# fizzy74/passport-zk-circuits

Hardware: AMD Instinct MI355X
Metric: registerIdentityBuilder witnesses/sec, batch=4096, 1 & 8 MI355X; % HBM roofline (higher is better)
Workload: dtype bn254_fr (u32 limbs)

## Files before the change

passport-zk-circuits_amd/csrc/builder_ecdsa.cpp:

```cpp
#include "builder_impl.hpp"
#include "ec_walk.hpp"

namespace pzk {

namespace {

struct EcSym { int idx = -1; };

struct EcProgCtx {
  using V = EcSym;
  uint32_t* d;
  uint32_t size;
  uint32_t n = 0;
  bool bad = false;
  uint32_t& at(uint32_t off) {
    static uint32_t sink;
    if (off >= size) { bad = true; return sink; }
    return d[off];
  }
  V put(uint32_t off, const V&) { at(off) = ecd(ECD_COPY, n); return V{(int)n++}; }
  V put_hidden(const V&) { return V{(int)n++}; }
  void cp(uint32_t off, const V& v) {
    if (v.idx < 0) bad = true;
    else at(off) = ecd(ECD_COPY, (uint32_t)v.idx);
// ... 22 lines not shown
  void check_one(const V&) const {}
  int nl = 4;
  void div_signed(const V*, int, int MCN, V& sign, V* k) const {
    sign = {};
    for (int i = 0; i < MCN - nl + 1; i++) k[i] = {};
  }
  void divmod_n(const V*, V* q, V* r) const {
    for (int i = 0; i < nl + 1; i++) q[i] = {};
    for (int i = 0; i < nl; i++) r[i] = {};
  }
};

template <int CV>
bool ec_program(int t, std::vector<uint32_t>& P, uint32_t& n) {
  const uint32_t size = ec_type_size(EC_GEO[CV], t);
  P.assign(size, ecd(ECD_ZERO, 0));
  EcProgCtx c{P.data(), size};
  c.nl = EC_GEO[CV].nl;
  EcWalk<EcProgCtx, CV> walk(c);
  walk.run(t);
  n = c.n;
  return !c.bad;
}

uint32_t sz_n2b(int L) { return 2 * L + 1; }

}

bool ec_programs(Layout& L, std::string& why) {
  const int cv = L.reg.ec_curve;
  const EcGeo& G = EC_GEO[cv];
  L.ec_prog.clear();
  for (int t = 0; t < ECT_N; t++) {
    std::vector<uint32_t> P;
    uint32_t n = 0;
    const bool ok = cv == 0 ? ec_program<0>(t, P, n) : cv == 1 ? ec_program<1>(t, P, n) : cv == 2 ? ec_program<2>(t, P, n)
                                                                                         : ec_program<3>(t, P, n);
    if (!ok || n > EC_TABLE_MAX[cv]) {
      why = "internal: ECDSA table program " + std::to_string(t) +
            (!ok ? " addresses a signal outside its block" : " too large (" + std::to_string(n) + " entries)");
      return false;
    }
    L.ec_prog_off[t] = (uint32_t)L.ec_prog.size();
    L.ec_tab_n[t] = n;
    L.ec_prog.insert(L.ec_prog.end(), P.begin(), P.end());
  }
  L.ec_tab_off.clear();
  for (int i = 0; i < ECT_N; i++) L.ec_ops[i].clear();
  uint32_t off = 0;
  for (int t = 0; t < G.n_ops + EC_N_MM; t++) {
    const int type = t >= G.n_ops ? ECT_MM : ec_op_is_dbl(G, t) ? ECT_DBL : ECT_ADD;
    L.ec_tab_off.push_back(off);
    L.ec_ops[type].push_back(t);
    off += L.ec_tab_n[type];
  }
  L.ec_tab_entries = off;
  return true;
}

void ec_verify_regions(Builder& b, int cv, int IN_PK, int IN_SIG, int J_SA) {
  const EcGeo& G = EC_GEO[cv];
  const int N = G.nl, CS = G.cs, F = G.fb, P2 = 2 * N;
  auto ect = [&](int t, int type) { b.region(RK_ECT, ec_type_size(G, type), {t, type}); };
  auto ecop = [&](int op) { ect(op, ec_op_is_dbl(G, op) ? ECT_DBL : ECT_ADD); };
  b.region(RK_INCOPY, P2, {IN_PK});
  b.region(RK_INCOPY, P2, {IN_SIG});
  b.region(RK_DIGEST, F, {J_SA});
  b.region(RK_INCOPY, P2, {IN_PK});
  b.region(RK_INCOPY, P2, {IN_SIG});
  b.region(RK_DIGEST, F, {J_SA});
  b.region(RK_HCHUNK, N, {J_SA, N, CS});
  b.region(RK_EC_CONST, N, {EC_K_ONE});
  b.region(RK_EC_CONST, N, {EC_K_ORDER});
  b.region(RK_EC_U64, N, {G.c_sinv});
  for (int i = 0; i < N; i++) b.region(RK_BITS2NUM, sz_n2b(CS), {CS, 1, i * CS + CS - 1, -1, J_SA});
  b.region(RK_EC_CONST, N, {EC_K_ORDER});
  b.region(RK_EC_U64, N, {G.c_sinv});
  b.region(RK_INCOPY, N, {IN_SIG + N});
  b.region(RK_EC_CONST, N, {EC_K_ORDER});
  ect(G.n_ops + EC_MM_INV, ECT_MM);
  ect(G.n_ops + EC_MM_U1, ECT_MM);
  ect(G.n_ops + EC_MM_U2, ECT_MM);
  b.region(RK_EC_U64, P2, {G.c_gm_rp + P2 * (G.parts - 2)});
  b.region(RK_EC_U64, N, {G.c_u1});
  b.region(RK_EC_GM_RCC, (uint64_t)G.parts * 256 * P2);
  b.region(RK_EC_U64, G.parts * P2, {G.c_gm_ap});
  b.region(RK_VALUE, 4 * G.parts * P2, {-2});
  b.region(RK_EC_U64, (G.parts - 1) * P2, {G.c_gm_rp});
  b.region(RK_VALUE, P2, {-2});
  for (int i = 0; i < N; i++) b.region(RK_EC_N2B, sz_n2b(CS), {0, G.c_u1 + i, CS});
  b.region(RK_EC_B2N8, G.parts * 17, {G.c_u1});
  b.region(RK_EC_CONST, P2, {EC_K_DUMMY});
  ecop(EC_OP_SD);
  b.region(RK_EC_GM_EQ, (uint64_t)G.parts * 256 * 6);
  b.region(RK_EC_GM_SUM, (uint64_t)G.parts * P2 * 512);
  for (int i = 0; i < G.parts - 1; i++) {
    ecop(ec_op_gm_add(i));
    b.region(RK_EC_GM_STEP, 4 * 6 + 2 * P2 * 6, {i});
  }
  b.region(RK_EC_U64, P2, {G.c_sm_rp + P2 * G.wins});
  b.region(RK_INCOPY, P2, {IN_PK});
  b.region(RK_EC_U64, N, {G.c_u2});
  b.region(RK_EC_SBITS, F, {G.c_u2});
  b.region(RK_EC_U64, (G.wins + 1) * P2, {G.c_sm_rp});
  b.region(RK_EC_U64, G.wins * P2, {G.c_sm_ap});
  b.region(RK_EC_U64, 16 * P2, {G.c_pre});
  b.region(RK_INCOPY, P2, {IN_PK});
// ... 23 lines not shown
```

passport-zk-circuits_amd/csrc/ec_common.hpp:

```cpp
#pragma once
#include <hip/hip_runtime.h>
#include <stdint.h>

namespace pzk {

constexpr int EC_N_CURVES = 4;
constexpr int EC_MAXN = 7;
__host__ __device__ constexpr int ec_curve_of_sig(int sig) {
  return sig == 20 ? 0 : sig == 21 ? 1 : sig == 24 ? 2 : sig == 25 ? 3 : -1;
}
constexpr int EC_NL[EC_N_CURVES] = {4, 4, 7, 6};
constexpr int EC_CS[EC_N_CURVES] = {64, 64, 32, 64};

constexpr uint64_t EC_CURVE_K[EC_N_CURVES][5][2 * EC_MAXN] = {
    {{18446744073709551612ull, 4294967295ull, 0ull, 18446744069414584321ull},
     {4309448131093880907ull, 7285987128567378166ull, 12964664127075681980ull, 6540974713487397863ull},
     {18446744073709551615ull, 4294967295ull, 0ull, 18446744069414584321ull},
     {17562291160714782033ull, 13611842547513532036ull, 18446744073709551615ull, 18446744069414584320ull},
     {4148137498610012746ull, 51237685452122967ull, 6555942389409504868ull, 799804747332166731ull,
      13395177781894339167ull, 1107697421929919296ull, 6228258783500845564ull, 11862546499924939746ull}},
    {{16810331318623712729ull, 18122579188607900780ull, 17219079075415130087ull, 9032542404991529047ull},
     {7767825457231955894ull, 10773760575486288334ull, 17523706096862592191ull, 2800214691157789508ull},
     {2311270323689771895ull, 7943213001558335528ull, 4496292894210231666ull, 12248480212390422972ull},
     {10384753744809580199ull, 10104242082523752183ull, 4496292894210231665ull, 12248480212390422972ull},
// ... 48 lines not shown
  const int P2 = 2 * N;
  g.c_sinv = 0; g.c_u1 = N; g.c_u2 = 2 * N; g.c_h = 3 * N;
  g.c_mm = 4 * N;
  g.c_gm_ap = g.c_mm + 4 * P2;
  g.c_gm_rp = g.c_gm_ap + g.parts * P2;
  g.c_pre = g.c_gm_rp + (g.parts - 1) * P2;
  g.c_sm_ap = g.c_pre + 16 * P2;
  g.c_sm_rp = g.c_sm_ap + g.wins * P2;
  g.c_rec = g.c_sm_rp + (g.wins + 1) * P2;
  g.rec_words = 3 * P2;
  g.core_words = g.c_rec + g.n_ops * g.rec_words;
  g.i_sm_zr = 4 * (g.parts - 1);
  g.i_sm_za = g.i_sm_zr + g.wins;
  g.n_inv = g.i_sm_za + g.wins - 1;
  g.n_pts = g.parts + (g.parts - 1) + 16 + g.wins + (g.wins + 1);
  g.jw = (g.fb + 63) / 64;
  g.j_op = (3 * g.jw + 2) & ~1;
  g.j_pts = g.n_ops * g.j_op;
  g.jac_words = g.j_pts + (g.n_pts + 1) / 2;
  g.sz_poncurve = P2 + 3 * ec_bmo(N, N) + ec_bmo(2 * N - 1, N) + ec_bizmp(cs, N, 3 * cs + 2 * N, 3 * N - 2, 3 * N);
  g.sz_pontangent = 4 * N + ec_bmo(N, N) + (2 * (2 * N - 1) + 1) + (2 * (2 * N - 1) + N) + 4 * N + ec_bmo(2 * N - 1, N) +
                    (2 * N + 1) + 3 * N + ec_bmo(N, N) + ec_bizmp(cs, N, 3 * cs + 2 * N, 3 * N - 2, 3 * N + 1);
  g.sz_ponline = 6 * N + 3 * N + 3 * 4 * N + 2 * ec_bmo(N, N) + ec_bizmp(cs, N, 2 * cs + 2 * N, 2 * N - 1, 2 * N + 1);
  g.sz_dbl = 4 * N + g.sz_pontangent + g.sz_poncurve;
  g.sz_add = 6 * N + g.sz_poncurve + g.sz_ponline;
  g.sz_blet = 1 + 2 * N + N + N * ((3 + ec_n2b(cs + 1)) + 6);
  g.sz_mm = (N + 1) + N + 3 * N + ec_bmo(N, N) + N * ec_n2b(cs) + (1 + 2 * N + g.sz_blet) + ec_bmneq(N + 1, N) +
            ec_bisz(cs, 2 * cs + ec_log_ceil(2 * N), 2 * N - 1);
  return g;
}
constexpr EcGeo EC_GEO[EC_N_CURVES] = {ec_geo_make(4, 64), ec_geo_make(4, 64), ec_geo_make(7, 32), ec_geo_make(6, 64)};
static_assert(EC_GEO[0].n_ops == 362 && EC_GEO[2].n_ops == 318 && EC_GEO[3].n_ops == 538, "EC op counts");

constexpr int EC_OP_SD = 0;
__host__ __device__ constexpr int ec_op_gm_add(int i) { return 1 + i; }
__host__ __device__ constexpr int ec_op_pre(const EcGeo& G, int i) { return G.parts + (i - 2); }
__host__ __device__ constexpr int ec_op_sm_dbl(const EcGeo& G, int d) { return G.op_sm0 + (d / 4) * 5 + (d % 4); }
__host__ __device__ constexpr int ec_op_sm_add(const EcGeo& G, int a) { return G.op_sm0 + a * 5 + 4; }
__host__ __device__ constexpr bool ec_op_is_dbl(const EcGeo& G, int op) {
  return op == EC_OP_SD || (op >= G.parts && op < G.op_sm0 && (op - G.parts) % 2 == 0) ||
         (op >= G.op_sm0 && op < G.op_final && (op - G.op_sm0) % 5 != 4);
}
enum { EC_MM_INV = 0, EC_MM_U1 = 1, EC_MM_U2 = 2, EC_MM_XN = 3, EC_N_MM = 4 };

enum : uint32_t { ECD_ZERO = 0, ECD_COPY = 1, ECD_BIT = 2, ECD_MASK = 3 };
__host__ __device__ constexpr uint32_t ecd(uint32_t op, uint32_t idx, uint32_t bit = 0) {
  return (op << 29) | (bit << 20) | idx;
}
enum EcType { ECT_DBL = 0, ECT_ADD = 1, ECT_MM = 2, ECT_N = 3 };
__host__ __device__ constexpr uint32_t ec_type_size(const EcGeo& G, int t) {
  return t == ECT_DBL ? G.sz_dbl : t == ECT_ADD ? G.sz_add : G.sz_mm;
}
constexpr uint32_t EC_TABLE_MAX[EC_N_CURVES] = {640, 640, 1600, 1216};

#ifndef PZK_EC_CURVE
#define PZK_EC_CURVE 0
#endif
#if PZK_EC_CURVE == 0
#define PZK_EC_NS ec_c0
#elif PZK_EC_CURVE == 1
#define PZK_EC_NS ec_c1
#elif PZK_EC_CURVE == 2
#define PZK_EC_NS ec_c2
#else
#define PZK_EC_NS ec_c3
#endif
inline namespace PZK_EC_NS {
static constexpr int EC_CV = PZK_EC_CURVE;
static constexpr EcGeo ECG = EC_GEO[EC_CV];
static constexpr const uint64_t (&EC_A)[2 * EC_MAXN] = EC_CURVE_K[EC_CV][EC_K_A];
static constexpr const uint64_t (&EC_B)[2 * EC_MAXN] = EC_CURVE_K[EC_CV][EC_K_B];
static constexpr const uint64_t (&EC_P)[2 * EC_MAXN] = EC_CURVE_K[EC_CV][EC_K_P];
static constexpr const uint64_t (&EC_N)[2 * EC_MAXN] = EC_CURVE_K[EC_CV][EC_K_ORDER];
static constexpr const uint64_t (&EC_D)[2 * EC_MAXN] = EC_CURVE_K[EC_CV][EC_K_DUMMY];
}

}
```

passport-zk-circuits_amd/csrc/ec_core.hpp:

```cpp
#pragma once
#include "ec_common.hpp"
#include "ec_walk.hpp"
#include "fr.hpp"
#include "layout.hpp"
#include "core_util.hpp"
#include "mapsink.hpp"
#include "bufs.hpp"
#include "ec_emit.hpp"

namespace pzk {
inline namespace PZK_EC_NS {

static constexpr int NL = ECG.nl, CS = ECG.cs, P2 = 2 * ECG.nl;
static constexpr int NW = (ECG.fb + 31) / 32, JW = ECG.jw;
static constexpr uint64_t CS_MASK = CS == 64 ? ~0ull : (1ull << CS) - 1;

struct I256 { uint32_t w[8]; };
__device__ __forceinline__ I256 i_u64(uint64_t x) {
  I256 r; r.w[0] = (uint32_t)x; r.w[1] = (uint32_t)(x >> 32);
#pragma unroll
  for (int i = 2; i < 8; i++) r.w[i] = 0;
  return r;
}
__device__ __forceinline__ I256 i_pow2(int k) {
// ... 92 lines not shown
      } else break;
    }
    uint64_t carry = 0, borrow = 0;
#pragma unroll
    for (int i = 0; i < NB; i++) {
      uint64_t pl = qhat * v[i], ph = __umul64hi(qhat, v[i]);
      pl += carry; ph += pl < carry;
      uint64_t t = u[i + j] - pl;
      uint64_t b1 = u[i + j] < pl;
      uint64_t t2 = t - borrow;
      b1 += t < borrow;
      u[i + j] = t2; borrow = b1; carry = ph;
    }
    uint64_t t = u[j + NB] - carry, b1 = u[j + NB] < carry;
    uint64_t t2 = t - borrow; b1 += t < borrow;
    u[j + NB] = t2;
    if (b1) {
      qhat--;
      uint64_t c = 0;
#pragma unroll
      for (int i = 0; i < NB; i++) {
        uint64_t s1 = u[i + j] + v[i], c1 = s1 < v[i];
        uint64_t s2 = s1 + c; c1 += s2 < c;
        u[i + j] = s2; c = c1;
      }
      u[j + NB] += c;
    }
    q[j] = qhat;
  }
#pragma unroll
  for (int i = 0; i < NB; i++) r[i] = (u[i] >> s) | (s ? u[i + 1] << (64 - s) : 0);
}
__device__ __forceinline__ void chunks_to_words(const uint64_t* ch, int n, uint64_t* w, int nw) {
  for (int i = 0; i < nw; i++) w[i] = 0;
  for (int i = 0; i < n; i++) w[(CS * i) >> 6] |= ch[i] << ((CS * i) & 63);
}
__device__ __forceinline__ uint64_t word_chunk(const uint64_t* w, int i) {
  return (w[(CS * i) >> 6] >> ((CS * i) & 63)) & CS_MASK;
}
static constexpr int PWORDS = (ECG.fb + 63) / 64;
__device__ __forceinline__ void const_words(const uint64_t* ch, uint64_t* w) { chunks_to_words(ch, NL, w, PWORDS); }

template <int AW32>
__device__ __forceinline__ void acc_signed(uint32_t* acc, const I256& v, int i) {
  const int off = (CS / 32) * i;
  const uint32_t ext = i_is_neg(v) ? ~0u : 0u;
  uint64_t c = 0;
  for (int j = 0; off + j < AW32; j++) {
    const uint64_t s = (uint64_t)acc[off + j] + (j < 8 ? v.w[j] : ext) + c;
    acc[off + j] = (uint32_t)s; c = s >> 32;
  }
}

struct EcTabCtx {
  using V = I256;
  uint4* tab;
  uint32_t n;
  const uint64_t* rp;
  int32_t err;
  __device__ void fail(int32_t code) { if (!err || code < err) err = code; }
  __device__ void store(const V& v) {
    I256 f = i_to_fr(v);
    tab[2 * n] = make_uint4(f.w[0], f.w[1], f.w[2], f.w[3]);
    tab[2 * n + 1] = make_uint4(f.w[4], f.w[5], f.w[6], f.w[7]);
    n++;
  }
  __device__ V put(uint32_t, const V& v) { store(v); return v; }
  __device__ V put_hidden(const V& v) { store(v); return v; }
  __device__ void cp(uint32_t, const V&) {}
  __device__ void bits(uint32_t, const V& v, int L) { if (!i_fits(v, L)) fail(ST_NUM2BITS); }
  __device__ void masks(uint32_t, const V&, int) {}
  __device__ V u64(uint64_t x) const { return i_u64(x); }
  __device__ V pow2(int k) const { return i_pow2(k); }
  __device__ V add(const V& a, const V& b) const { return i_add(a, b); }
  __device__ V sub(const V& a, const V& b) const { return i_sub(a, b); }
  __device__ V mul(const V& a, const V& b) const { return i_mul(a, b); }
  __device__ V neg(const V& a) const { return i_neg(a); }
  __device__ V sel(const V& c, const V& a, const V& b) const { return c.w[0] ? a : b; }
  __device__ V is_zero(const V& a) const { return i_u64(i_is_zero(a) ? 1 : 0); }
  __device__ V bit(const V& a, int b) const { return i_u64(i_bit(a, b)); }
  __device__ V shr_exact(const V& t, int) {
    I256 r; const uint32_t s = i_is_neg(t) ? ~0u : 0u;
    if (CS == 64) {
      if (t.w[0] | t.w[1]) fail(ST_BIGISZERO);
      return i_shr64(t);
    }
    if (t.w[0]) fail(ST_BIGISZERO);
#pragma unroll
    for (int i = 0; i < 8; i++) r.w[i] = i + 1 < 8 ? t.w[i + 1] : s;
    return r;
  }
  __device__ V inv_fr(const V& d) const {
    fr x = fr_mul_fast(i_as_fr(i_to_fr(d)), fr_const(R2_));
    fr y = fr_from_mont_fast(fr_inv<true>(x));
    I256 r;
    for (int i = 0; i < 8; i++) r.w[i] = y.v[i];
    return r;
  }
  __device__ void check_zero(const V& v) { if (!i_is_zero(v)) fail(ST_BIGISZERO); }
  __device__ void check_one(const V& v) {
    if (!i_is_zero(i_sub(v, i_u64(1)))) fail(ST_BIGMOD_GT);
  }
  __device__ void div_signed(const V* in, int CN, int MCN, V& sign, V* k) {
    constexpr int AW = ((3 * NL + 1) * CS + 63) / 64 + 2, AW32 = 2 * AW;
    uint32_t acc[AW32];
    for (int i = 0; i < AW32; i++) acc[i] = 0;
    for (int i = 0; i < CN; i++) acc_signed<AW32>(acc, in[i], i);
    const bool pos = !(acc[AW32 - 1] >> 31);
    if (!pos) {
      uint64_t c = 1;
      for (int i = 0; i < AW32; i++) { const uint64_t x = (uint64_t)(uint32_t)~acc[i] + c; acc[i] = (uint32_t)x; c = x >> 32; }
    }
    uint64_t a[AW], pw[PWORDS], q[AW], r[PWORDS];
    for (int i = 0; i < AW; i++) { a[i] = (uint64_t)acc[2 * i + 1] << 32 | acc[2 * i]; q[i] = 0; }
    const_words(EC_P, pw);
    const int na = (MCN * CS + 63) / 64;
    mp_divmod<PWORDS>(a, na < PWORDS ? PWORDS : na, pw, q, r);
    sign = i_u64(pos ? 1 : 0);
    for (int i = 0; i < MCN - NL + 1; i++) k[i] = i_u64(word_chunk(q, i));
// ... 548 lines not shown
    if (ec_op_is_dbl(ECG, it)) { for (int i = 0; i < P2; i++) rc[P2 + i] = 0; }
    else aff((int32_t)(uint32_t)(hh >> 32), rc + P2);
  } else if (it < ECG.n_ops + ECG.n_pts) {
    const int idx = it - ECG.n_ops;
    aff(reinterpret_cast<const int32_t*>(J + ECG.j_pts)[idx], C + ec_pt_base(idx));
  } else {
    const uint64_t* x1 = C + ECG.c_rec + ECG.rec_words * ECG.op_final + 2 * P2;
    eW xm = m_reduce<ModN>(ew_from_chunks(x1).v, 0);
    uint64_t xr[NL];
    ew_to_chunks(xm, xr);
    bool ok = true;
    for (int i = 0; i < NL; i++) {
      ok &= xr[i] == *reinterpret_cast<const uint64_t*>(row + 32ull * (L.reg.in_sig + i));
      C[ECG.c_mm + P2 * EC_MM_XN + i] = x1[i];
      C[ECG.c_mm + P2 * EC_MM_XN + NL + i] = i == 0 ? 1 : 0;
    }
    if (!ok && status) lane_status(status + w, ST_ECDSA_R);
  }
}

__device__ __forceinline__ fr ec_inv_diff(const uint64_t* ec_core, uint32_t w, int j) {
  const uint64_t* C = ec_core + (size_t)w * ECG.core_words;
  const uint64_t dx = EC_D[0];
  fr d;
  if (j < ECG.i_sm_zr) {
    const int i = j >> 2, k = j & 3;
    const uint64_t lx = i == 0 ? C[ECG.c_gm_ap] : C[ECG.c_gm_rp + P2 * (i - 1)], rx = C[ECG.c_gm_ap + P2 * (i + 1)];
    const uint64_t sdx = C[ECG.c_rec + ECG.rec_words * EC_OP_SD + 2 * P2];
    d = fr_diff_u64(k < 2 ? lx : rx, (k & 1) ? sdx : dx);
  } else if (j < ECG.i_sm_za) {
    d = fr_diff_u64(dx, C[ECG.c_sm_rp + P2 * (j - ECG.i_sm_zr)]);
  } else {
    d = fr_diff_u64(dx, C[ECG.c_sm_ap + P2 * (j - ECG.i_sm_za + 1)]);
  }
  return d;
}

__global__ void __launch_bounds__(64) k_ec_inv(const uint64_t* ec_core, fr* ec_inv, uint32_t batch) {
  const uint32_t gid = blockIdx.x * blockDim.x + threadIdx.x;
  const uint32_t w = gid / ECG.n_inv;
  const int j = (int)(gid % ECG.n_inv);
  const bool live = w < batch;
  fr d = fr_zero();
  if (live) d = ec_inv_diff(ec_core, w, j);
  const fr a = fr_is_zero(d) ? fr_mont_one() : fr_mul_fast(d, fr_const(R2_));
  fr others, total;
  fr_group_others<64>(a, others, total);
  const fr r = fr_mul_fast(fr_inv<true>(total), others);
  if (live) ec_inv[(size_t)w * ECG.n_inv + j] = fr_is_zero(d) ? d : fr_from_mont_fast(r);
}


template <int TYPE>
__global__ void __launch_bounds__(64) k_ec_table(DevLayout L, const int32_t* ops, const uint64_t* ec_core, uint8_t* ec_tab,
                                                 int32_t* status, uint32_t batch) {
  const uint32_t w = blockIdx.x * blockDim.x + threadIdx.x;
  if (w >= batch) return;
  const int t = ops[blockIdx.y];
  const uint64_t* C = ec_core + (size_t)w * ECG.core_words;
  const uint64_t* rec = t < ECG.n_ops ? C + ECG.c_rec + ECG.rec_words * t : C + ECG.c_mm + P2 * (t - ECG.n_ops);
  uint4* tab = reinterpret_cast<uint4*>(ec_tab + 32ull * ((size_t)w * L.ec_tab_entries + L.ec_tab_off[t]));
  EcTabCtx c{tab, 0, rec, 0};
  EcWalk<EcTabCtx, EC_CV> walk(c);
  walk.run(TYPE);
  if (c.err && status) lane_status(status + w, c.err);
}

__device__ __forceinline__ uint4 ect_value(const uint4* tab, uint32_t d, uint32_t half) {
  const uint32_t op = d >> 29, bit = (d >> 20) & 511u, idx = d & 0xfffffu;
  if (op == ECD_ZERO) return make_uint4(0u, 0u, 0u, 0u);
  if (op == ECD_COPY) return tab[2 * idx + half];
  if (op == ECD_BIT) {
    if (half) return make_uint4(0u, 0u, 0u, 0u);
    const uint4 q = tab[2 * idx + (bit >> 7)];
    const uint32_t k = (bit >> 5) & 3u, wv = k == 0 ? q.x : k == 1 ? q.y : k == 2 ? q.z : q.w;
    return make_uint4((wv >> (bit & 31u)) & 1u, 0u, 0u, 0u);
  }
  const uint4 q = tab[2 * idx + half];
  const int nb = (int)bit + 1, lo = 128 * (int)half;
  auto mw = [&](uint32_t x, int k) -> uint32_t {
    const int b0 = lo + 32 * k;
    return nb >= b0 + 32 ? x : nb <= b0 ? 0u : (x & ((1u << (nb - b0)) - 1u));
  };
  return make_uint4(mw(q.x, 0), mw(q.y, 1), mw(q.z, 2), mw(q.w, 3));
}

constexpr int ECT_NT = EC_TABLE_MAX[EC_CV] > 1024 ? 512 : 256;
template <int MM, int ECT_U>
__global__ void __launch_bounds__(ECT_NT) k_emit_ect(DevLayout L, const Work* work, const uint8_t* ec_tab, uint8_t* wtns,
                                                  size_t stride, int prefetch, uint32_t wpb, uint32_t batch) {
  __shared__ uint4 tab[2 * EC_TABLE_MAX[EC_CV]];
  constexpr int TL = (2 * EC_TABLE_MAX[EC_CV] + ECT_NT - 1) / ECT_NT;
  const Work wk = work[blockIdx.x];
  const uint32_t wb = blockIdx.y * wpb, we = wb + wpb < batch ? wb + wpb : batch;
  const Region R = L.regions[wk.region];
  const int t = R.a[0], type = R.a[1];
  const uint32_t n2 = 2 * L.ec_tab_n[type];
  typedef uint32_t u32x4 __attribute__((ext_vector_type(4)));
  const u32x4* tab0 = reinterpret_cast<const u32x4*>(ec_tab + 32ull * L.ec_tab_off[t]);
  u32x4* tabv = reinterpret_cast<u32x4*>(tab);
  const size_t tab_stride = 2ull * L.ec_tab_entries;
  uint32_t ti[TL];
#pragma unroll
  for (int k = 0; k < TL; k++) ti[k] = threadIdx.x + k * ECT_NT < n2 ? threadIdx.x + k * ECT_NT : 0u;
  u32x4 tv[TL];
  const uint64_t g = R.off + wk.start;
  const uint32_t* o0_prog = L.ec_prog + L.ec_prog_off[type] + wk.start;
  const DescRun dr0 = desc_run<MM>(L, wtns, stride, wb, wk, g, o0_prog);
  const uint32_t* prog = dr0.prog;
  const uint32_t tot = 2 * dr0.count, step = ECT_U * blockDim.x;
  uint32_t d[ECT_U], dn[ECT_U];
  auto load = [&](uint32_t base, uint32_t* dd) {
#pragma unroll
    for (int k = 0; k < ECT_U; k++) {
      const uint32_t h = base + k * blockDim.x;
      dd[k] = h < tot ? prog[h >> 1] : 0u;
    }
  };
  load(threadIdx.x, dn);
#pragma unroll
  for (int k = 0; k < TL; k++) tv[k] = tab0[wb * tab_stride + ti[k]];
  for (uint32_t w = wb; w < we; w++) {
    if (w > wb) __syncthreads();
#pragma unroll
    for (int k = 0; k < TL; k++) tabv[ti[k]] = tv[k];
    __syncthreads();
    const bool more_w = w + 1 < we;
    const size_t nt = (more_w ? w + 1 : w) * tab_stride;
#pragma unroll
    for (int k = 0; k < TL; k++) tv[k] = tab0[nt + ti[k]];
    const OutRow out = desc_run<MM>(L, wtns, stride, w, wk, g, o0_prog).out;
    for (uint32_t base = threadIdx.x; base < tot; base += step) {
#pragma unroll
      for (int k = 0; k < ECT_U; k++) d[k] = dn[k];
      const bool more = base + step < tot || more_w;
      const uint32_t nbase = base + step < tot ? base + step : threadIdx.x;
      if (prefetch && more) load(nbase, dn);
#pragma unroll
      for (int k = 0; k < ECT_U; k++) {
        const uint32_t h = base + k * blockDim.x;
        store_half<MAP_O0>(out, h, h < tot ? ect_value(tab, d[k], h & 1) : make_uint4(0u, 0u, 0u, 0u), h < tot);
      }
      if (!prefetch && more) load(nbase, dn);
    }
  }
}

template <int MM>
__global__ void __launch_bounds__(256) k_emit_ecr(DevLayout L, const Work* work, Bufs B) {
  constexpr int MAXP = 4;
  __shared__ uint64_t ap[MAXP][P2];
  __shared__ uint32_t bt[MAXP];
  __shared__ fr inv[256];
  __shared__ uint4 stage[2 * 256];
  const Work wk = work[blockIdx.x];
  const uint32_t w = blockIdx.y;
  const Region R = L.regions[wk.region];
  const uint64_t* C = B.ec_core + (size_t)w * ECG.core_words;
  const uint32_t per = R.kind == RK_EC_GM_RCC ? 256u * P2 : R.kind == RK_EC_GM_EQ ? 256u * 6 : 512u * P2;
  const uint32_t i0 = wk.start / per;
  for (uint32_t t = threadIdx.x; t < MAXP * P2; t += blockDim.x) {
    const uint32_t k = t / P2, q = t % P2, i = i0 + k;
    if (i < (uint32_t)ECG.parts) ap[k][q] = C[ECG.c_gm_ap + P2 * i + q];
  }
  if (threadIdx.x < MAXP && i0 + threadIdx.x < (uint32_t)ECG.parts) {
    uint64_t u1[NL];
    for (int k = 0; k < NL; k++) u1[k] = C[ECG.c_u1 + k];
    bt[threadIdx.x] = (uint32_t)sc_byte(u1, (int)(i0 + threadIdx.x));
  }
  if (R.kind == RK_EC_GM_EQ) inv[threadIdx.x] = B.inv_small[threadIdx.x];
  __syncthreads();
  const OutRow out = out_row(L, B.wtns, B.stride, w, R.off + wk.start);
  if (R.kind == RK_EC_GM_RCC) {
    emit_run<MM>(out, wk.count, stage, [&](uint32_t q0) -> El {
      const uint32_t s = wk.start + q0, k = s / (256u * P2) - i0, j = (s / P2) % 256u, q = s % P2;
      return el_u64(bt[k] == j ? ap[k][q] : 0ull);
    });
  } else if (R.kind == RK_EC_GM_EQ) {
    emit_run<MM>(out, wk.count, stage, [&](uint32_t q0) -> El {
      const uint32_t s = wk.start + q0, blk = s / 6, e = s % 6, k = (blk >> 8) - i0, j = blk & 255u, b = bt[k];
      const int d = (int)b - (int)j;
      return iseq_sig((int)e, j, b, d == 0 ? fr_zero() : d > 0 ? inv[d] : fr_sub(fr_zero(), inv[-d]));
    });
// ... 12 lines not shown
```

passport-zk-circuits_amd/csrc/kernels_ec.hip:

```cpp
#include <hip/hip_runtime.h>
#include <stdlib.h>

#include "bufs.hpp"
#include "ec_core.hpp"
#include "kernels.hpp"

namespace pzk {
inline namespace PZK_EC_NS {

#define HIP_TRY(x) do { hipError_t e_ = (x); if (e_ != hipSuccess) return e_; } while (0)

hipError_t launch_ec_core_cv(const DevLayout& L, const uint8_t* inputs, const uint32_t* sha_core, uint64_t* ec_core,
                          uint64_t* ec_jac, fr* ec_inv, int32_t* status, uint32_t batch, hipStream_t st) {
  hipLaunchKernelGGL(k_ec_scalars, dim3((batch + 63) / 64), dim3(64), 0, st, L, inputs, sha_core, ec_core, status, batch);
  HIP_TRY(hipGetLastError());
  hipLaunchKernelGGL(k_ec_chain, dim3((2 * batch + 63) / 64), dim3(64), 0, st, L, inputs, ec_core, ec_jac, batch);
  HIP_TRY(hipGetLastError());
  hipLaunchKernelGGL(k_ec_final, dim3((batch + 63) / 64), dim3(64), 0, st, L, inputs, ec_jac, batch);
  HIP_TRY(hipGetLastError());
  hipLaunchKernelGGL(k_ec_affine, dim3((batch * EC_AFF_GROUPS + 63) / 64), dim3(64), 0, st, ec_core, ec_jac, status,
                     batch);
  HIP_TRY(hipGetLastError());
  hipLaunchKernelGGL(k_ec_link, dim3((batch * EC_LINK_ITEMS + 63) / 64), dim3(64), 0, st, L, inputs, ec_core, ec_jac,
                     status, batch);
  HIP_TRY(hipGetLastError());
  hipLaunchKernelGGL(k_ec_inv, dim3((batch * ECG.n_inv + 63) / 64), dim3(64), 0, st, ec_core, ec_inv, batch);
  return hipGetLastError();
}

hipError_t launch_ec_table_cv(const DevLayout& L, int type, const int32_t* ops, uint32_t n_ops, const uint64_t* ec_core,
                           uint8_t* ec_tab, int32_t* status, uint32_t batch, hipStream_t st) {
  if (n_ops == 0) return hipSuccess;
  dim3 g((batch + 63) / 64, n_ops);
  switch (type) {
    case ECT_DBL: hipLaunchKernelGGL(k_ec_table<ECT_DBL>, g, dim3(64), 0, st, L, ops, ec_core, ec_tab, status, batch); break;
    case ECT_ADD: hipLaunchKernelGGL(k_ec_table<ECT_ADD>, g, dim3(64), 0, st, L, ops, ec_core, ec_tab, status, batch); break;
    default: hipLaunchKernelGGL(k_ec_table<ECT_MM>, g, dim3(64), 0, st, L, ops, ec_core, ec_tab, status, batch); break;
  }
  return hipGetLastError();
}

hipError_t launch_emit_ect_cv(const DevLayout& L, const Work* work, uint32_t n_work, const Bufs& B, uint32_t batch,
                           hipStream_t st) {
  if (n_work == 0) return hipSuccess;
  static const int prefetch = getenv("PZK_ECT_PREFETCH") ? atoi(getenv("PZK_ECT_PREFETCH")) : 1;
  static const int u = getenv("PZK_ECT_U") ? atoi(getenv("PZK_ECT_U")) : 16;
  auto kern = L.keep.bits ? k_emit_ect<MAP_DIRECT, 16>
              : u == 16 ? k_emit_ect<MAP_O0, 16> : u == 32 ? k_emit_ect<MAP_O0, 32> : k_emit_ect<MAP_O0, 8>;
  static const uint32_t wpb = getenv("PZK_ECT_WPB") ? (uint32_t)atoi(getenv("PZK_ECT_WPB")) : 4u;
  if (wpb < 1 || wpb > 64) return hipErrorInvalidValue;
  hipLaunchKernelGGL(kern, dim3(n_work, (batch + wpb - 1) / wpb), dim3(ECT_NT), 0, st, L, work, B.ec_tab, B.wtns,
                     B.stride, prefetch, wpb, batch);
  return hipGetLastError();
}

hipError_t launch_emit_ecr_cv(const DevLayout& L, const Work* work, uint32_t n_work, const Bufs& B, uint32_t batch,
                              hipStream_t st) {
  if (n_work == 0) return hipSuccess;
  hipLaunchKernelGGL((L.keep.bits ? k_emit_ecr<MAP_DIRECT> : k_emit_ecr<MAP_O0>), dim3(n_work, batch), dim3(256), 0, st, L, work, B);
  return hipGetLastError();
}

}

#if PZK_EC_CURVE == 0
#define PZK_EC_DECL(ns)                                                                                                   \
  namespace ns {                                                                                                        \
  hipError_t launch_ec_core_cv(const DevLayout& L, const uint8_t* inputs, const uint32_t* sha_core, uint64_t* ec_core,  \
                               uint64_t* ec_jac, fr* ec_inv, int32_t* status, uint32_t batch, hipStream_t st);          \
  hipError_t launch_ec_table_cv(const DevLayout& L, int type, const int32_t* ops, uint32_t n_ops,                       \
                                const uint64_t* ec_core, uint8_t* ec_tab, int32_t* status, uint32_t batch,              \
                                hipStream_t st);                                                                        \
  hipError_t launch_emit_ect_cv(const DevLayout& L, const Work* work, uint32_t n_work, const Bufs& B, uint32_t batch,   \
                                hipStream_t st);                                                                        \
  hipError_t launch_emit_ecr_cv(const DevLayout& L, const Work* work, uint32_t n_work, const Bufs& B, uint32_t batch,   \
                                hipStream_t st);                                                                        \
  }
PZK_EC_DECL(ec_c1)
PZK_EC_DECL(ec_c2)
PZK_EC_DECL(ec_c3)
#undef PZK_EC_DECL

#define PZK_EC_DISPATCH(call)                         \
  switch (L.reg.ec_curve) {                           \
    case 1: return ec_c1::call;                       \
    case 2: return ec_c2::call;                       \
    case 3: return ec_c3::call;                       \
    default: return ec_c0::call;                      \
  }
hipError_t launch_ec_core(const DevLayout& L, const uint8_t* inputs, const uint32_t* sha_core, uint64_t* ec_core,
                          uint64_t* ec_jac, fr* ec_inv, int32_t* status, uint32_t batch, hipStream_t st) {
  PZK_EC_DISPATCH(launch_ec_core_cv(L, inputs, sha_core, ec_core, ec_jac, ec_inv, status, batch, st))
}
hipError_t launch_ec_table(const DevLayout& L, int type, const int32_t* ops, uint32_t n_ops, const uint64_t* ec_core,
                           uint8_t* ec_tab, int32_t* status, uint32_t batch, hipStream_t st) {
  PZK_EC_DISPATCH(launch_ec_table_cv(L, type, ops, n_ops, ec_core, ec_tab, status, batch, st))
}
hipError_t launch_emit_ect(const DevLayout& L, const Work* work, uint32_t n_work, const Bufs& B, uint32_t batch,
                           hipStream_t st) {
  PZK_EC_DISPATCH(launch_emit_ect_cv(L, work, n_work, B, batch, st))
}
hipError_t launch_emit_ecr(const DevLayout& L, const Work* work, uint32_t n_work, const Bufs& B, uint32_t batch,
// ... 7 lines not shown
```

passport-zk-circuits_amd/csrc/probe/probe.h:

```cpp
#pragma once
#include <stdint.h>

#ifdef __cplusplus
extern "C" {
#endif

#define PZK_PROBE_MAX_CASES 4096

enum {
  PFR_ADD = 0, PFR_SUB, PFR_REDUCE_ONCE, PFR_GEQ_P , PFR_MUL, PFR_SQR, PFR_MUL_FAST, PFR_FROM_MONT,
  PFR_FROM_MONT_FAST, PFR_TO_MONT, PFR_TO_MONT_IN, PFR_INV, PFR_INV_FAST, PFR_INV_SW, PFR_INV_SW_FAST,
  PFR_FROM_I128 , PFR_N_OPS
};
int pzk_probe_fr(int op, const uint32_t* a, const uint32_t* b, uint32_t* out, int n);
int pzk_probe_fr_batch_inv(const uint32_t* x, uint32_t* out, int n, int m);

enum {
  PFQ_MUL = 0, PFQ_MUL64, PFQ_MULQ, PFQ_DOT1, PFQ_DOT2, PFQ_DOT3, PFQ_CANON, PFQ_GEQ_P, PFQ_ADD_RAW, PFQ_N_OPS
};
int pzk_probe_fq(int op, const uint32_t* a, const uint32_t* b, const uint32_t* k, uint32_t* out, uint32_t* out_canon,
                 int n);

enum { PDIV_DIVLU = 0, PDIV_PREINV = 1 };
int pzk_probe_div64(int op, const uint64_t* u1, const uint64_t* u0, const uint64_t* v, uint64_t* q, uint64_t* r, int n);
int pzk_probe_kd_div(const uint64_t* a, const int* na, int sa, const uint64_t* b, const int* nb, int sb, uint64_t* q,
                     uint64_t* r, int n);

enum { PEC_MUL = 0, PEC_ADD, PEC_SUB, PEC_TO, PEC_FROM, PEC_INV, PEC_N_OPS };
int pzk_probe_ec_nw(int cv);
int pzk_probe_ec_pwords(int cv);
int pzk_probe_ec_field(int cv, int mod_n, int op, const uint32_t* a, const uint32_t* b, uint32_t* out, int n);
int pzk_probe_ec_divmod(int cv, int mod_n, const uint64_t* a, const int* na, uint64_t* q, uint64_t* r, int n);

int pzk_probe_ntt(int inverse, int shift, int k, int batch, const int* split, int n_split, const uint32_t* in,
                  uint32_t* out, int on_device);
int pzk_probe_ntt_plan(int k, int* q, int* r);

#ifdef __cplusplus
}
#endif
```

passport-zk-circuits_amd/csrc/probe/probe_ec.hip:

```cpp
#include <hip/hip_runtime.h>

#include "../ec_core.hpp"
#include "probe_util.hpp"

namespace pzk {
inline namespace PZK_EC_NS {
using namespace pzkprobe;

template <class M, int OP>
__global__ void __launch_bounds__(64) k_probe_ec_field(const uint32_t* a, const uint32_t* b, uint32_t* out, int n) {
  const int c = blockIdx.x * 64 + threadIdx.x;
  if (c >= n) return;
  eW x, y, r;
  for (int i = 0; i < NW; i++) { x.v[i] = a[NW * c + i]; y.v[i] = b ? b[NW * c + i] : 0u; }
  if constexpr (OP == PEC_MUL) r = m_mul_inl<M>(x, y);
  else if constexpr (OP == PEC_ADD) r = m_add<M>(x, y);
  else if constexpr (OP == PEC_SUB) r = m_sub<M>(x, y);
  else if constexpr (OP == PEC_TO) r = m_to<M>(x);
  else if constexpr (OP == PEC_FROM) r = m_from<M>(x);
  else r = m_inv<M>(x);
  for (int i = 0; i < NW; i++) out[NW * c + i] = r.v[i];
}

__global__ void __launch_bounds__(64) k_probe_ec_divmod(int mod_n, const uint64_t* a, const int* na, uint64_t* q,
// ... 40 lines not shown
  if (bad_count(n) || !a || !na || !q || !r) return (int)hipErrorInvalidValue;
  for (int c = 0; c < n; c++)
    if (na[c] < PWORDS || na[c] > 31) return (int)hipErrorInvalidValue;
  if (n == 0) return 0;
  DBuf da, dna, dq, dr;
  PROBE_TRY(da.up(a, 8 * 32 * (size_t)n));
  PROBE_TRY(dna.up(na, sizeof(int) * (size_t)n));
  PROBE_TRY(dq.up(nullptr, 8 * 32 * (size_t)n));
  PROBE_TRY(dr.up(nullptr, 8 * (size_t)PWORDS * n));
  hipLaunchKernelGGL(k_probe_ec_divmod, dim3((n + 63) / 64), dim3(64), 0, 0, mod_n, da.as<uint64_t>(), dna.as<int>(),
                     dq.as<uint64_t>(), dr.as<uint64_t>(), n);
  PROBE_TRY(finish());
  PROBE_TRY(dq.down(q, 8 * 32 * (size_t)n));
  return (int)dr.down(r, 8 * (size_t)PWORDS * n);
}

}

#if PZK_EC_CURVE == 0
#define PZK_PROBE_DECL(ns)                                                                                 \
  namespace ns {                                                                                           \
  int probe_ec_nw_cv();                                                                                    \
  int probe_ec_pwords_cv();                                                                                \
  int probe_ec_field_cv(int mod_n, int op, const uint32_t* a, const uint32_t* b, uint32_t* out, int n);    \
  int probe_ec_divmod_cv(int mod_n, const uint64_t* a, const int* na, uint64_t* q, uint64_t* r, int n);    \
  }
PZK_PROBE_DECL(ec_c1)
PZK_PROBE_DECL(ec_c2)
PZK_PROBE_DECL(ec_c3)
#undef PZK_PROBE_DECL
#define PZK_PROBE_DISPATCH(call, bad) \
  switch (cv) {                        \
    case 0: return ec_c0::call;        \
    case 1: return ec_c1::call;        \
    case 2: return ec_c2::call;        \
    case 3: return ec_c3::call;        \
    default: return bad;               \
  }
#endif
}

#if PZK_EC_CURVE == 0
using namespace pzk;
extern "C" int pzk_probe_ec_nw(int cv) { PZK_PROBE_DISPATCH(probe_ec_nw_cv(), -1) }
extern "C" int pzk_probe_ec_pwords(int cv) { PZK_PROBE_DISPATCH(probe_ec_pwords_cv(), -1) }
extern "C" int pzk_probe_ec_field(int cv, int mod_n, int op, const uint32_t* a, const uint32_t* b, uint32_t* out, int n) {
  PZK_PROBE_DISPATCH(probe_ec_field_cv(mod_n, op, a, b, out, n), (int)hipErrorInvalidValue)
}
extern "C" int pzk_probe_ec_divmod(int cv, int mod_n, const uint64_t* a, const int* na, uint64_t* q, uint64_t* r, int n) {
  PZK_PROBE_DISPATCH(probe_ec_divmod_cv(mod_n, a, na, q, r, n), (int)hipErrorInvalidValue)
}
#undef PZK_PROBE_DISPATCH
#endif
```

Before: 85210.

## Compress ECDSA table storage into low plane plus sparse high plane with bitmasks

Changes the per-witness EC table layout from full 32-byte entries to a dense low 16-byte plane, a compacted high plane holding only entries with nonzero upper words, and per-16-entry bitmask/rank words. The emit kernel reconstructs entries with popcount ranks, prefetching masks two witnesses ahead. This cuts HBM traffic for the table write and read, since many field values are small, at the cost of extra index arithmetic and a dependent mask load. It also raises the default witnesses per block from 4 to 8, adds occupancy hints to the launch bounds, and adds a probe for round-trip testing of the layout.

Measured after the change: 84890. No clear change (-0.4%).

```diff
diff --git a/passport-zk-circuits_amd/csrc/builder_ecdsa.cpp b/passport-zk-circuits_amd/csrc/builder_ecdsa.cpp
--- a/passport-zk-circuits_amd/csrc/builder_ecdsa.cpp
+++ b/passport-zk-circuits_amd/csrc/builder_ecdsa.cpp
@@ -98,7 +98,7 @@
     const int type = t >= G.n_ops ? ECT_MM : ec_op_is_dbl(G, t) ? ECT_DBL : ECT_ADD;
     L.ec_tab_off.push_back(off);
     L.ec_ops[type].push_back(t);
-    off += L.ec_tab_n[type];
+    off += ec_tab_region(L.ec_tab_n[type]);
   }
   L.ec_tab_entries = off;
   return true;
diff --git a/passport-zk-circuits_amd/csrc/ec_common.hpp b/passport-zk-circuits_amd/csrc/ec_common.hpp
--- a/passport-zk-circuits_amd/csrc/ec_common.hpp
+++ b/passport-zk-circuits_amd/csrc/ec_common.hpp
@@ -124,6 +124,9 @@
   return t == ECT_DBL ? G.sz_dbl : t == ECT_ADD ? G.sz_add : G.sz_mm;
 }
 constexpr uint32_t EC_TABLE_MAX[EC_N_CURVES] = {640, 640, 1600, 1216};
+__host__ __device__ constexpr uint32_t ec_tab_pad(uint32_t n) { return (n + 7u) & ~7u; }
+__host__ __device__ constexpr uint32_t ec_tab_mask_lines(uint32_t n) { return (n + 511u) / 512u; }
+__host__ __device__ constexpr uint32_t ec_tab_region(uint32_t n) { return ec_tab_pad(n) + 4u * ec_tab_mask_lines(n); }
 
 #ifndef PZK_EC_CURVE
 #define PZK_EC_CURVE 0
diff --git a/passport-zk-circuits_amd/csrc/ec_core.hpp b/passport-zk-circuits_amd/csrc/ec_core.hpp
--- a/passport-zk-circuits_amd/csrc/ec_core.hpp
+++ b/passport-zk-circuits_amd/csrc/ec_core.hpp
@@ -168,19 +168,39 @@
   }
 }
 
+typedef uint32_t etw_v4 __attribute__((ext_vector_type(4)));
+struct EcTabWriter {
+  uint8_t* reg;
+  uint32_t n_pad;
+  uint32_t n, c1, mcur;
+  __device__ void init(uint8_t* region, uint32_t ntab) {
+    reg = region; n_pad = ec_tab_pad(ntab);
+    n = c1 = mcur = 0;
+  }
+  __device__ void push(const I256& f) {
+    const uint32_t wide = (f.w[4] | f.w[5] | f.w[6] | f.w[7]) != 0;
+    *reinterpret_cast<etw_v4*>(reg + 16ull * n) = (etw_v4){f.w[0], f.w[1], f.w[2], f.w[3]};
+    *reinterpret_cast<etw_v4*>(reg + 16ull * n_pad + 16ull * c1) = (etw_v4){f.w[4], f.w[5], f.w[6], f.w[7]};
+    c1 += wide;
+    mcur |= wide << (n & 15u);
+    n++;
+    if ((n & 15u) == 0) {
+      *reinterpret_cast<uint32_t*>(reg + 32ull * n_pad + 4ull * (n / 16 - 1)) = mcur;
+      mcur = c1 << 16;
+    }
+  }
+  __device__ void finish() {
+    if (n & 15u) *reinterpret_cast<uint32_t*>(reg + 32ull * n_pad + 4ull * (n / 16)) = mcur;
+  }
+};
+
 struct EcTabCtx {
   using V = I256;
-  uint4* tab;
-  uint32_t n;
+  EcTabWriter tw;
   const uint64_t* rp;
   int32_t err;
   __device__ void fail(int32_t code) { if (!err || code < err) err = code; }
-  __device__ void store(const V& v) {
-    I256 f = i_to_fr(v);
-    tab[2 * n] = make_uint4(f.w[0], f.w[1], f.w[2], f.w[3]);
-    tab[2 * n + 1] = make_uint4(f.w[4], f.w[5], f.w[6], f.w[7]);
-    n++;
-  }
+  __device__ void store(const V& v) { tw.push(i_to_fr(v)); }
   __device__ V put(uint32_t, const V& v) { store(v); return v; }
   __device__ V put_hidden(const V& v) { store(v); return v; }
   __device__ void cp(uint32_t, const V&) {}
@@ -835,17 +855,18 @@
 
 
 template <int TYPE>
-__global__ void __launch_bounds__(64) k_ec_table(DevLayout L, const int32_t* ops, const uint64_t* ec_core, uint8_t* ec_tab,
+__global__ void __launch_bounds__(64, 2) k_ec_table(DevLayout L, const int32_t* ops, const uint64_t* ec_core, uint8_t* ec_tab,
                                                  int32_t* status, uint32_t batch) {
   const uint32_t w = blockIdx.x * blockDim.x + threadIdx.x;
   if (w >= batch) return;
   const int t = ops[blockIdx.y];
   const uint64_t* C = ec_core + (size_t)w * ECG.core_words;
   const uint64_t* rec = t < ECG.n_ops ? C + ECG.c_rec + ECG.rec_words * t : C + ECG.c_mm + P2 * (t - ECG.n_ops);
-  uint4* tab = reinterpret_cast<uint4*>(ec_tab + 32ull * ((size_t)w * L.ec_tab_entries + L.ec_tab_off[t]));
-  EcTabCtx c{tab, 0, rec, 0};
+  EcTabCtx c{{}, rec, 0};
+  c.tw.init(ec_tab + 32ull * ((size_t)w * L.ec_tab_entries + L.ec_tab_off[t]), L.ec_tab_n[TYPE]);
   EcWalk<EcTabCtx, EC_CV> walk(c);
   walk.run(TYPE);
+  c.tw.finish();
   if (c.err && status) lane_status(status + w, c.err);
 }
 
@@ -869,24 +890,59 @@
 }
 
 constexpr int ECT_NT = EC_TABLE_MAX[EC_CV] > 1024 ? 512 : 256;
+
+template <int NT>
+struct EctLoader {
+  static constexpr int TE = (EC_TABLE_MAX[EC_CV] + NT - 1) / NT;
+  typedef uint32_t u32x4 __attribute__((ext_vector_type(4)));
+  const uint8_t* reg0;
+  size_t wbytes;
+  uint32_t n_pad;
+  uint32_t tid, n;
+  uint32_t mw[TE];
+  u32x4 lo[TE], hi[TE];
+  __device__ __forceinline__ void init(const uint8_t* region0, size_t witness_bytes, uint32_t entries, uint32_t thread) {
+    reg0 = region0; wbytes = witness_bytes; n = entries; n_pad = ec_tab_pad(n); tid = thread;
+  }
+  __device__ __forceinline__ uint32_t entry(int k) const { return tid + k * NT < n ? tid + k * NT : 0u; }
+  __device__ __forceinline__ void masks(uint32_t w) {
+    const uint32_t* m = reinterpret_cast<const uint32_t*>(reg0 + (size_t)w * wbytes + 32ull * n_pad);
+#pragma unroll
+    for (int k = 0; k < TE; k++) mw[k] = m[entry(k) >> 4];
+  }
+  __device__ __forceinline__ void planes(uint32_t w) {
+    const u32x4* p0 = reinterpret_cast<const u32x4*>(reg0 + (size_t)w * wbytes);
+    const u32x4* p1 = p0 + n_pad;
+#pragma unroll
+    for (int k = 0; k < TE; k++) {
+      const uint32_t e = entry(k), b = e & 15u, has = (mw[k] >> b) & 1u;
+      const uint32_t rank = (mw[k] >> 16) + (uint32_t)__popc(mw[k] & ((1u << b) - 1u));
+      lo[k] = p0[e];
+      hi[k] = (u32x4){0u, 0u, 0u, 0u};
+      if (has && rank < n_pad) hi[k] = p1[rank];
+    }
+  }
+  __device__ __forceinline__ void fill(uint4* tab) const {
+    u32x4* tv = reinterpret_cast<u32x4*>(tab);
+#pragma unroll
+    for (int k = 0; k < TE; k++) {
+      const uint32_t e = entry(k);
+      tv[2 * e] = lo[k];
+      tv[2 * e + 1] = hi[k];
+    }
+  }
+};
+
 template <int MM, int ECT_U>
-__global__ void __launch_bounds__(ECT_NT) k_emit_ect(DevLayout L, const Work* work, const uint8_t* ec_tab, uint8_t* wtns,
+__global__ void __launch_bounds__(ECT_NT, ECT_NT == 256 && ECT_U <= 16 ? 3 : 1) k_emit_ect(DevLayout L, const Work* work, const uint8_t* ec_tab, uint8_t* wtns,
                                                   size_t stride, int prefetch, uint32_t wpb, uint32_t batch) {
   __shared__ uint4 tab[2 * EC_TABLE_MAX[EC_CV]];
-  constexpr int TL = (2 * EC_TABLE_MAX[EC_CV] + ECT_NT - 1) / ECT_NT;
   const Work wk = work[blockIdx.x];
   const uint32_t wb = blockIdx.y * wpb, we = wb + wpb < batch ? wb + wpb : batch;
   const Region R = L.regions[wk.region];
   const int t = R.a[0], type = R.a[1];
-  const uint32_t n2 = 2 * L.ec_tab_n[type];
-  typedef uint32_t u32x4 __attribute__((ext_vector_type(4)));
-  const u32x4* tab0 = reinterpret_cast<const u32x4*>(ec_tab + 32ull * L.ec_tab_off[t]);
-  u32x4* tabv = reinterpret_cast<u32x4*>(tab);
-  const size_t tab_stride = 2ull * L.ec_tab_entries;
-  uint32_t ti[TL];
-#pragma unroll
-  for (int k = 0; k < TL; k++) ti[k] = threadIdx.x + k * ECT_NT < n2 ? threadIdx.x + k * ECT_NT : 0u;
-  u32x4 tv[TL];
+  EctLoader<ECT_NT> ld;
+  ld.init(ec_tab + 32ull * L.ec_tab_off[t], 32ull * L.ec_tab_entries, L.ec_tab_n[type], threadIdx.x);
   const uint64_t g = R.off + wk.start;
   const uint32_t* o0_prog = L.ec_prog + L.ec_prog_off[type] + wk.start;
   const DescRun dr0 = desc_run<MM>(L, wtns, stride, wb, wk, g, o0_prog);
@@ -900,18 +956,17 @@
       dd[k] = h < tot ? prog[h >> 1] : 0u;
     }
   };
+  ld.masks(wb);
   load(threadIdx.x, dn);
-#pragma unroll
-  for (int k = 0; k < TL; k++) tv[k] = tab0[wb * tab_stride + ti[k]];
+  ld.planes(wb);
+  ld.masks(wb + 1 < we ? wb + 1 : we - 1);
   for (uint32_t w = wb; w < we; w++) {
     if (w > wb) __syncthreads();
-#pragma unroll
-    for (int k = 0; k < TL; k++) tabv[ti[k]] = tv[k];
+    ld.fill(tab);
     __syncthreads();
     const bool more_w = w + 1 < we;
-    const size_t nt = (more_w ? w + 1 : w) * tab_stride;
-#pragma unroll
-    for (int k = 0; k < TL; k++) tv[k] = tab0[nt + ti[k]];
+    ld.planes(more_w ? w + 1 : w);
+    ld.masks(w + 2 < we ? w + 2 : we - 1);
     const OutRow out = desc_run<MM>(L, wtns, stride, w, wk, g, o0_prog).out;
     for (uint32_t base = threadIdx.x; base < tot; base += step) {
 #pragma unroll
diff --git a/passport-zk-circuits_amd/csrc/kernels_ec.hip b/passport-zk-circuits_amd/csrc/kernels_ec.hip
--- a/passport-zk-circuits_amd/csrc/kernels_ec.hip
+++ b/passport-zk-circuits_amd/csrc/kernels_ec.hip
@@ -47,7 +47,7 @@
   static const int u = getenv("PZK_ECT_U") ? atoi(getenv("PZK_ECT_U")) : 16;
   auto kern = L.keep.bits ? k_emit_ect<MAP_DIRECT, 16>
               : u == 16 ? k_emit_ect<MAP_O0, 16> : u == 32 ? k_emit_ect<MAP_O0, 32> : k_emit_ect<MAP_O0, 8>;
-  static const uint32_t wpb = getenv("PZK_ECT_WPB") ? (uint32_t)atoi(getenv("PZK_ECT_WPB")) : 4u;
+  static const uint32_t wpb = getenv("PZK_ECT_WPB") ? (uint32_t)atoi(getenv("PZK_ECT_WPB")) : 8u;
   if (wpb < 1 || wpb > 64) return hipErrorInvalidValue;
   hipLaunchKernelGGL(kern, dim3(n_work, (batch + wpb - 1) / wpb), dim3(ECT_NT), 0, st, L, work, B.ec_tab, B.wtns,
                      B.stride, prefetch, wpb, batch);
diff --git a/passport-zk-circuits_amd/csrc/probe/probe.h b/passport-zk-circuits_amd/csrc/probe/probe.h
--- a/passport-zk-circuits_amd/csrc/probe/probe.h
+++ b/passport-zk-circuits_amd/csrc/probe/probe.h
@@ -32,6 +32,10 @@
 int pzk_probe_ec_field(int cv, int mod_n, int op, const uint32_t* a, const uint32_t* b, uint32_t* out, int n);
 int pzk_probe_ec_divmod(int cv, int mod_n, const uint64_t* a, const int* na, uint64_t* q, uint64_t* r, int n);
 
+int pzk_probe_ectab_max(int cv);
+#define PZK_PROBE_ECTAB_GUARD (-2)
+int pzk_probe_ectab(int cv, const uint32_t* values, uint32_t* out, int n, int batch, int wpb);
+
 int pzk_probe_ntt(int inverse, int shift, int k, int batch, const int* split, int n_split, const uint32_t* in,
                   uint32_t* out, int on_device);
 int pzk_probe_ntt_plan(int k, int* q, int* r);
diff --git a/passport-zk-circuits_amd/csrc/probe/probe_ec.hip b/passport-zk-circuits_amd/csrc/probe/probe_ec.hip
--- a/passport-zk-circuits_amd/csrc/probe/probe_ec.hip
+++ b/passport-zk-circuits_amd/csrc/probe/probe_ec.hip
@@ -116,3 +116,5 @@
 }
 #undef PZK_PROBE_DISPATCH
 #endif
+
+#include "probe_ectab.hip"
diff --git a/passport-zk-circuits_amd/csrc/probe/probe_ectab.hip b/passport-zk-circuits_amd/csrc/probe/probe_ectab.hip
--- /dev/null
+++ b/passport-zk-circuits_amd/csrc/probe/probe_ectab.hip
@@ -0,0 +1,100 @@
+
+namespace pzk {
+inline namespace PZK_EC_NS {
+
+__global__ void __launch_bounds__(64) k_probe_ectab_write(const uint32_t* values, uint8_t* region0, size_t wbytes,
+                                                          uint32_t n, uint32_t batch) {
+  const uint32_t w = blockIdx.x * blockDim.x + threadIdx.x;
+  if (w >= batch) return;
+  EcTabWriter tw;
+  tw.init(region0 + (size_t)w * wbytes, n);
+  for (uint32_t i = 0; i < n; i++) {
+    I256 f;
+    for (int k = 0; k < 8; k++) f.w[k] = values[((size_t)w * n + i) * 8 + k];
+    tw.push(f);
+  }
+  tw.finish();
+}
+
+__global__ void __launch_bounds__(ECT_NT) k_probe_ectab_read(const uint8_t* region0, size_t wbytes, uint32_t n,
+                                                             uint32_t wpb, uint32_t batch, uint4* out) {
+  __shared__ uint4 tab[2 * EC_TABLE_MAX[EC_CV]];
+  const uint32_t wb = blockIdx.x * wpb, we = wb + wpb < batch ? wb + wpb : batch;
+  EctLoader<ECT_NT> ld;
+  ld.init(region0, wbytes, n, threadIdx.x);
+  ld.masks(wb);
+  ld.planes(wb);
+  ld.masks(wb + 1 < we ? wb + 1 : we - 1);
+  for (uint32_t w = wb; w < we; w++) {
+    if (w > wb) __syncthreads();
+    ld.fill(tab);
+    __syncthreads();
+    ld.planes(w + 1 < we ? w + 1 : w);
+    ld.masks(w + 2 < we ? w + 2 : we - 1);
+    for (uint32_t i = threadIdx.x; i < 2 * n; i += blockDim.x) out[(size_t)w * 2 * n + i] = tab[i];
+  }
+}
+
+int probe_ectab_max_cv() { return (int)EC_TABLE_MAX[EC_CV]; }
+
+int probe_ectab_cv(const uint32_t* values, uint32_t* out, int n, int batch, int wpb) {
+  using namespace pzkprobe;
+  if (!values || !out || n < 1 || n > (int)EC_TABLE_MAX[EC_CV] || batch < 1 || batch > PZK_PROBE_MAX_CASES || wpb < 1 ||
+      wpb > 64)
+    return (int)hipErrorInvalidValue;
+  const size_t region = 32ull * ec_tab_region((uint32_t)n), wbytes = region + 128, vbytes = 32ull * n * batch;
+  DBuf dv, dt, dout;
+  PROBE_TRY(dv.up(values, vbytes));
+  PROBE_TRY(dt.up(nullptr, wbytes * batch));
+  PROBE_TRY(hipMemset(dt.p, 0xA5, wbytes * batch));
+  PROBE_TRY(dout.up(nullptr, vbytes));
+  hipLaunchKernelGGL(k_probe_ectab_write, dim3((batch + 63) / 64), dim3(64), 0, 0, dv.as<uint32_t>(), dt.as<uint8_t>(),
+                     wbytes, (uint32_t)n, (uint32_t)batch);
+  PROBE_TRY(finish());
+  hipLaunchKernelGGL(k_probe_ectab_read, dim3((batch + wpb - 1) / wpb), dim3(ECT_NT), 0, 0, dt.as<uint8_t>(), wbytes,
+                     (uint32_t)n, (uint32_t)wpb, (uint32_t)batch, dout.as<uint4>());
+  PROBE_TRY(finish());
+  uint8_t guard[128];
+  for (int w = 0; w < batch; w++) {
+    PROBE_TRY(hipMemcpy(guard, dt.as<uint8_t>() + wbytes * w + region, 128, hipMemcpyDeviceToHost));
+    for (int i = 0; i < 128; i++)
+      if (guard[i] != 0xA5) return PZK_PROBE_ECTAB_GUARD;
+  }
+  return (int)dout.down(out, vbytes);
+}
+
+}
+
+#if PZK_EC_CURVE == 0
+#define PZK_PROBE_ECTAB_DECL(ns)                                                               \
+  namespace ns {                                                                               \
+  int probe_ectab_max_cv();                                                                    \
+  int probe_ectab_cv(const uint32_t* values, uint32_t* out, int n, int batch, int wpb);       \
+  }
+PZK_PROBE_ECTAB_DECL(ec_c1)
+PZK_PROBE_ECTAB_DECL(ec_c2)
+PZK_PROBE_ECTAB_DECL(ec_c3)
+#undef PZK_PROBE_ECTAB_DECL
+#endif
+}
+
+#if PZK_EC_CURVE == 0
+extern "C" int pzk_probe_ectab_max(int cv) {
+  switch (cv) {
+    case 0: return pzk::ec_c0::probe_ectab_max_cv();
+    case 1: return pzk::ec_c1::probe_ectab_max_cv();
+    case 2: return pzk::ec_c2::probe_ectab_max_cv();
+    case 3: return pzk::ec_c3::probe_ectab_max_cv();
+    default: return -1;
+  }
+}
+extern "C" int pzk_probe_ectab(int cv, const uint32_t* values, uint32_t* out, int n, int batch, int wpb) {
+  switch (cv) {
+    case 0: return pzk::ec_c0::probe_ectab_cv(values, out, n, batch, wpb);
+    case 1: return pzk::ec_c1::probe_ectab_cv(values, out, n, batch, wpb);
+    case 2: return pzk::ec_c2::probe_ectab_cv(values, out, n, batch, wpb);
+    case 3: return pzk::ec_c3::probe_ectab_cv(values, out, n, batch, wpb);
+    default: return (int)hipErrorInvalidValue;
+  }
+}
+#endif
```
